# yenanjing/mmEgo

Measured on AMD Instinct MI355X. Metric: train frames/sec (Upper+Lower U+L step, B=64/GPU, T=8, 128 pts), higher is better.
Workload: dtype f32; 1 GPU; U+L step (Train_Upper + Train_Lower train_once bodies), B=64/GPU T=8 N=128, fp32, dropout live, two concurrent HIP-graph branches; global_batch=64, seq_len=8, points=128, parallelism=dp1

## Files before the change

mmego_amd/csrc/gemm.hip:

```cpp
#include <stdlib.h>

#include "common.h"

#include "gemm_tile.h"
#include "lstm_cell.h"
#include "tile_order.h"

struct GemmP {
  const float* A;
  const float* B;
  float* C;
  const float* bias;
  long sam, sak, sbk, sbn, scm, scn;
  long sAb, sBb, sCb, sCs, sBiasb;
  int M, N, K;
  int nsplit, kchunk;
  int relu, accumulate;
  int avec, bvec;
  const float* cmul;
  float* asum;
  const float* cb_dout[2]; long cb_dos;
  const float* cb_gst[2]; const float* cb_cst[2]; const float* cb_cprev[2];
  float* cb_dc[2]; float* cb_dg[2]; long cb_dgs;
};

#define LD64 68
constexpr long GEMM_TILE_MIN_OTHER = 256;
constexpr int GEMM_KQ_MAX = 512;

template <bool A_KC, bool B_KC, int BK>
__global__ __launch_bounds__(256) void gemm64_kernel(GemmP p) {
  constexpr int EL = BK / 4;
  __shared__ float As[BK][LD64];
  __shared__ float Bs[BK][LD64];
  const int tid = threadIdx.x, lane = tid & 63, wave = tid >> 6;
  const int wm = wave & 1, wn = wave >> 1;
  const int batch = blockIdx.z / p.nsplit, split = blockIdx.z % p.nsplit;
  const int m0 = blockIdx.x * 64, n0 = blockIdx.y * 64;
  const float* A = p.A + (long)batch * p.sAb;
  const float* B = p.B + (long)batch * p.sBb;
  const int kbeg = split * p.kchunk;
  const int kend = min(p.K, kbeg + p.kchunk);

  const int am = A_KC ? (tid >> 2) : (tid & 63), bn = B_KC ? (tid >> 2) : (tid & 63);
  const int akb = A_KC ? (tid & 3) * 4 : (tid >> 6), bkb = B_KC ? (tid & 3) * 4 : (tid >> 6);
  const float* Arow = A + (long)min(m0 + am, p.M - 1) * p.sam;
  const float* Bcol = B + (long)min(n0 + bn, p.N - 1) * p.sbn;
  const bool avec = A_KC && p.avec, bvec = B_KC && p.bvec;

  float ra[EL], rb[EL];
#define G64_PIN(v) asm volatile("" : "+v"(v))
#define G64_LOAD1(R, PTR, SK, KC, VEC, KB, k0)                                                                \
  do {                                                                                                        \
    const bool whole_ = (k0) + BK <= kend;                                                       \
    if (KC) {                                                                                                 \
      if ((VEC) && whole_) {                                                                                  \
        _Pragma("unroll") for (int g = 0; g < EL / 4; ++g) {                                                  \
          const f32x4 v = *reinterpret_cast<const f32x4*>((PTR) + (k0) + (KB) + 16 * g);                      \
          R[4 * g] = v.x; R[4 * g + 1] = v.y; R[4 * g + 2] = v.z; R[4 * g + 3] = v.w;                         \
        }                                                                                                     \
      } else {                                                                                                \
        _Pragma("unroll") for (int j = 0; j < EL; ++j)                                                        \
          R[j] = (PTR)[(long)min((k0) + (KB) + 16 * (j >> 2) + (j & 3), kend - 1) * (SK)];                    \
        if (!whole_) {                                                                                        \
          _Pragma("unroll") for (int j = 0; j < EL; ++j) {                                                    \
            G64_PIN(R[j]);                                                                                    \
            R[j] = ((k0) + (KB) + 16 * (j >> 2) + (j & 3) < kend) ? R[j] : 0.0f;                              \
          }                                                                                                   \
        }                                                                                                     \
      }                                                                                                       \
    } else {                                                                                                  \
      _Pragma("unroll") for (int j = 0; j < EL; ++j) R[j] = (PTR)[(long)min((k0) + (KB) + 4 * j, kend - 1) * (SK)]; \
      if (!whole_) {                                                                                          \
        _Pragma("unroll") for (int j = 0; j < EL; ++j) {                                                      \
          G64_PIN(R[j]);                                                                                      \
          R[j] = ((k0) + (KB) + 4 * j < kend) ? R[j] : 0.0f;                                                  \
        }                                                                                                     \
      }                                                                                                       \
    }                                                                                                         \
  } while (0)
#define G64_LOAD(k0)                                                                                          \
  do {                                                                                                        \
    G64_LOAD1(ra, Arow, p.sak, A_KC, avec, akb, k0);                                                          \
    G64_LOAD1(rb, Bcol, p.sbk, B_KC, bvec, bkb, k0);                                                          \
  } while (0)

  f32x16 acc = {0};
  if (kbeg < kend) G64_LOAD(kbeg);
  for (int k0 = kbeg; k0 < kend; k0 += BK) {
    __syncthreads();
#pragma unroll
    for (int j = 0; j < EL; ++j) {
      As[A_KC ? akb + 16 * (j >> 2) + (j & 3) : akb + 4 * j][am] = ra[j];
      Bs[B_KC ? bkb + 16 * (j >> 2) + (j & 3) : bkb + 4 * j][bn] = rb[j];
    }
    __syncthreads();
    if (k0 + BK < kend) G64_LOAD(k0 + BK);
    const int r = lane & 31, h = lane >> 5;
#pragma unroll
    for (int kk = 0; kk < BK; kk += 2) {
      float a = As[kk + h][wm * 32 + r];
      float b = Bs[kk + h][wn * 32 + r];
      acc = __builtin_amdgcn_mfma_f32_32x32x2f32(a, b, acc, 0, 0, 0);
    }
  }
#undef G64_LOAD
#undef G64_LOAD1
#undef G64_PIN

  const int col = n0 + wn * 32 + (lane & 31);
  if (col >= p.N) return;
  float* C = p.C + (long)batch * p.sCb + (long)split * p.sCs;
  const float bv = (p.bias && p.nsplit == 1) ? p.bias[(long)batch * p.sBiasb + col] : 0.0f;
  const int rbase = m0 + wm * 32 + 4 * (lane >> 5);
  const bool final_ = p.nsplit == 1;
  float old[16], cm[16];
  if (final_ && p.accumulate) {
#pragma unroll
    for (int reg = 0; reg < 16; ++reg) {
      const int row = rbase + (reg & 3) + 8 * (reg >> 2);
      old[reg] = C[(long)(row < p.M ? row : p.M - 1) * p.scm + (long)col * p.scn];
    }
  }
  if (final_ && p.cmul) {
    const float* cmp = p.cmul + (C - p.C);
#pragma unroll
    for (int reg = 0; reg < 16; ++reg) {
      const int row = rbase + (reg & 3) + 8 * (reg >> 2);
      cm[reg] = cmp[(long)(row < p.M ? row : p.M - 1) * p.scm + (long)col * p.scn];
    }
  }
#pragma unroll
  for (int reg = 0; reg < 16; ++reg) {
    float v = acc[reg] + bv;
    if (final_) {
      if (p.relu == 1) v = fmaxf(v, 0.0f);
      if (p.accumulate) { asm volatile("" : "+v"(old[reg])); v += old[reg]; }
      if (p.cmul) { asm volatile("" : "+v"(cm[reg])); v = p.relu == 2 ? (cm[reg] > 0.f ? v : 0.f) : v * cm[reg]; }
    }
    acc[reg] = v;
  }
  float* cp = C + (long)rbase * p.scm + (long)col * p.scn;
  if (m0 + wm * 32 + 32 <= p.M) {
#pragma unroll
    for (int reg = 0; reg < 16; ++reg) cp[(long)((reg & 3) + 8 * (reg >> 2)) * p.scm] = acc[reg];
  } else {
#pragma unroll
    for (int reg = 0; reg < 16; ++reg)
      if (rbase + (reg & 3) + 8 * (reg >> 2) < p.M) cp[(long)((reg & 3) + 8 * (reg >> 2)) * p.scm] = acc[reg];
  }
}

template <bool A_KC, bool B_KC>
__device__ __forceinline__ void gemm32kq_body(const GemmP& p, const int bx, const int by, const int bz) {
  __shared__ float red[4][32][33];
  const int tid = threadIdx.x, lane = tid & 63, wave = tid >> 6;
  const int r = lane & 31, h = lane >> 5;
  const int batch = bz / p.nsplit, split = bz % p.nsplit;
  const int m0 = bx * 32, n0 = by * 32;
  const float* A = p.A + (long)batch * p.sAb;
  const float* B = p.B + (long)batch * p.sBb;
  const int kbeg0 = split * p.kchunk;
  const int kend0 = min(p.K, kbeg0 + p.kchunk);
  const int kq = (((kend0 - kbeg0) + 3) / 4 + 31) / 32 * 32;
  const int kbeg = kbeg0 + wave * kq;
  const int kend = min(kend0, kbeg + kq);
  const float* Arow = A + (long)min(m0 + r, p.M - 1) * p.sam;
  const float* Bcol = B + (long)min(n0 + r, p.N - 1) * p.sbn;
  const bool avec = A_KC && p.avec, bvec = B_KC && p.bvec;

  float ra[16], rb[16], na[16], nb[16];
#define KQ_PIN(v) asm volatile("" : "+v"(v))
#define KQ_LOAD1(R, PTR, SK, VEC, k0)                                                                         \
  do {                                                                                                        \
    const int kl = (k0) + 16 * h;                                                                             \
    if ((VEC) && (k0) + 32 <= kend) {                                                                         \
      _Pragma("unroll") for (int g = 0; g < 4; ++g) {                                                         \
        const f32x4 v = *reinterpret_cast<const f32x4*>((PTR) + kl + 4 * g);                                  \
        R[4 * g] = v.x; R[4 * g + 1] = v.y; R[4 * g + 2] = v.z; R[4 * g + 3] = v.w;                           \
      }                                                                                                       \
    } else {                                                                                                  \
      _Pragma("unroll") for (int s_ = 0; s_ < 16; ++s_) R[s_] = (PTR)[(long)min(kl + s_, kend - 1) * (SK)];   \
      if ((k0) + 32 > kend) {                                                                                 \
        _Pragma("unroll") for (int s_ = 0; s_ < 16; ++s_) { KQ_PIN(R[s_]); R[s_] = (kl + s_ < kend) ? R[s_] : 0.0f; } \
      }                                                                                                       \
    }                                                                                                         \
  } while (0)
#define KQ_LOAD(RA, RB, k0)                                                                                   \
  do {                                                                                                        \
    KQ_LOAD1(RA, Arow, p.sak, avec, k0);                                                                      \
    KQ_LOAD1(RB, Bcol, p.sbk, bvec, k0);                                                                      \
  } while (0)

  f32x16 acc = {0};
  const bool want_asum = p.asum != nullptr && by == 0;
  float asum = 0.f;
  if (kbeg < kend) {
    KQ_LOAD(ra, rb, kbeg);
    for (int k0 = kbeg; k0 < kend; k0 += 32) {
      const bool more = k0 + 32 < kend;
      if (more) KQ_LOAD(na, nb, k0 + 32);
      if (want_asum) {
#pragma unroll
        for (int s_ = 0; s_ < 16; ++s_) asum += ra[s_];
      }
#pragma unroll
      for (int s_ = 0; s_ < 16; ++s_) acc = __builtin_amdgcn_mfma_f32_32x32x2f32(ra[s_], rb[s_], acc, 0, 0, 0);
      if (more) {
#pragma unroll
        for (int s_ = 0; s_ < 16; ++s_) { ra[s_] = na[s_]; rb[s_] = nb[s_]; }
      }
    }
  }
#undef KQ_LOAD
#undef KQ_LOAD1
#undef KQ_PIN
#pragma unroll
  for (int reg = 0; reg < 16; ++reg) red[wave][(reg & 3) + 8 * (reg >> 2) + 4 * h][r] = acc[reg];
  __shared__ float ared[4][2][32];
  if (want_asum) ared[wave][h][r] = asum;
  __syncthreads();
  if (want_asum && tid < 32 && m0 + tid < p.M) {
    float v = 0.f;
#pragma unroll
    for (int w = 0; w < 4; ++w) v += ared[w][0][tid] + ared[w][1][tid];
    if (p.nsplit == 1) {
      float* dst = p.asum + (long)batch * p.M + m0 + tid;
      *dst = p.accumulate ? *dst + v : v;
    } else {
      p.asum[((long)split * (gridDim.z / p.nsplit) + batch) * p.M + m0 + tid] = v;
    }
  }
  if (p.cb_dg[0]) {
    const int col = tid & 31, H = p.N, d = batch;
    float dh[4], gi[4], gf[4], gg[4], go[4], cc[4], cp[4], dcin[4];
#pragma unroll
    for (int e = 0; e < 4; ++e) {
      const int row = (tid >> 5) + 8 * e;
      const long r = m0 + row, j = n0 + col, i = r * H + j;
      const float rec = ((red[0][row][col] + red[1][row][col]) + red[2][row][col]) + red[3][row][col];
      const float* gs = p.cb_gst[d] + r * 4 * H + j;
      dh[e] = p.cb_dout[d][r * p.cb_dos + j] + rec;
      gi[e] = gs[0]; gf[e] = gs[H]; gg[e] = gs[2 * H]; go[e] = gs[3 * H];
      cc[e] = p.cb_cst[d][i];
      cp[e] = p.cb_cprev[d] ? p.cb_cprev[d][i] : 0.f;
      dcin[e] = p.cb_dc[d][i];
    }
    LstmCellGrad o[4];
#pragma unroll
    for (int e = 0; e < 4; ++e) {
      asm volatile("" : "+v"(gi[e]), "+v"(gf[e]), "+v"(gg[e]), "+v"(go[e]), "+v"(cc[e]), "+v"(cp[e]), "+v"(dcin[e]), "+v"(dh[e]));
      o[e] = lstm_cell_bwd(gi[e], gf[e], gg[e], go[e], tanhf(cc[e]), cp[e], dcin[e], dh[e]);
    }
#pragma unroll
    for (int e = 0; e < 4; ++e) {
      const int row = (tid >> 5) + 8 * e;
      const long r = m0 + row, j = n0 + col;
      float* dg = p.cb_dg[d] + r * p.cb_dgs + j;
      dg[0] = o[e].di; dg[H] = o[e].df; dg[2 * H] = o[e].dg; dg[3 * H] = o[e].dout;
      p.cb_dc[d][r * H + j] = o[e].dcprev;
    }
    return;
  }
  float* C = p.C + (long)batch * p.sCb + (long)split * p.sCs;
  const bool final_ = p.nsplit == 1;
  const int col = tid & 31, colc = n0 + col < p.N ? n0 + col : p.N - 1;
  long off[4];
  float v[4], old[4], cm[4], bv = 0.f;
#pragma unroll
  for (int e = 0; e < 4; ++e) {
    const int row = (tid >> 5) + 8 * e;
    v[e] = ((red[0][row][col] + red[1][row][col]) + red[2][row][col]) + red[3][row][col];
    off[e] = (long)(m0 + row < p.M ? m0 + row : p.M - 1) * p.scm + (long)colc * p.scn;
  }
  if (final_ && p.bias) bv = p.bias[(long)batch * p.sBiasb + colc];
  if (final_ && p.accumulate) {
#pragma unroll
    for (int e = 0; e < 4; ++e) old[e] = C[off[e]];
  }
  if (final_ && p.cmul) {
    const float* cmp = p.cmul + (C - p.C);
#pragma unroll
    for (int e = 0; e < 4; ++e) cm[e] = cmp[off[e]];
  }
  if (final_) {
#pragma unroll
    for (int e = 0; e < 4; ++e) {
      float x = v[e] + bv;
      if (p.relu == 1) x = fmaxf(x, 0.0f);
      if (p.accumulate) { asm volatile("" : "+v"(old[e])); x += old[e]; }
      if (p.cmul) { asm volatile("" : "+v"(cm[e])); x = p.relu == 2 ? (cm[e] > 0.f ? x : 0.f) : x * cm[e]; }
      v[e] = x;
    }
  }
  if (m0 + 32 <= p.M && n0 + 32 <= p.N) {
#pragma unroll
    for (int e = 0; e < 4; ++e) C[off[e]] = v[e];
  } else {
#pragma unroll
    for (int e = 0; e < 4; ++e)
      if (m0 + (tid >> 5) + 8 * e < p.M && n0 + col < p.N) C[off[e]] = v[e];
  }
}

template <bool A_KC, bool B_KC>
__global__ __launch_bounds__(256) void gemm32kq_kernel(GemmP p) {
  gemm32kq_body<A_KC, B_KC>(p, blockIdx.x, blockIdx.y, blockIdx.z);
}

#define GEMM_GROUP_MAX 10
struct GemmGroup { GemmP p[GEMM_GROUP_MAX]; int zend[GEMM_GROUP_MAX]; int n; };
template <bool A_KC, bool B_KC>
__global__ __launch_bounds__(256) void gemm32kq_group_kernel(GemmGroup g) {
  int i = 0;
  const int z = blockIdx.z;
  while (i + 1 < g.n && z >= g.zend[i]) ++i;
  const int z0 = i ? g.zend[i - 1] : 0;
  const GemmP& p = g.p[i];
  if ((int)blockIdx.x * 32 >= p.M || (int)blockIdx.y * 32 >= p.N) return;
  gemm32kq_body<A_KC, B_KC>(p, blockIdx.x, blockIdx.y, z - z0);
}

#define SKR_OUT 16
#define SKR_LANES 16
__global__ __launch_bounds__(256) void splitk_reduce_kernel(const float* __restrict__ ws, float* C, const float* bias, int nsplit,
                                                            int nbatch, int M, int N, long scm, long scn, long sCb,
                                                            int relu, int accumulate, const float* __restrict__ asum_ws,
                                                            float* asum_out) {
  __shared__ float sh[SKR_LANES][SKR_OUT + 1];
  long total = (long)nbatch * M * N;
  const int o = threadIdx.x & (SKR_OUT - 1), kg = threadIdx.x / SKR_OUT;
  long i = (long)blockIdx.x * SKR_OUT + o;
  const long cblocks = (total + SKR_OUT - 1) / SKR_OUT;
  const bool is_asum = (long)blockIdx.x >= cblocks;
  if (is_asum) {
    i = ((long)blockIdx.x - cblocks) * SKR_OUT + o;
    total = (long)nbatch * M;
    ws = asum_ws;
  }
  float s = 0.0f;
  if (i < total) {
    const float* src = ws + i;
    int k = kg;
#pragma unroll 1
    for (; k + 7 * SKR_LANES < nsplit; k += 8 * SKR_LANES) {
      float v[8];
#pragma unroll
      for (int u = 0; u < 8; ++u) v[u] = src[(long)(k + u * SKR_LANES) * total];
#pragma unroll
      for (int u = 0; u < 8; ++u) s += v[u];
    }
    for (; k < nsplit; k += SKR_LANES) s += src[(long)k * total];
  }
  sh[kg][o] = s;
  __syncthreads();
  if (kg == 0 && i < total) {
    s = sh[0][o];
#pragma unroll
    for (int g = 1; g < SKR_LANES; ++g) s += sh[g][o];
    if (is_asum) {
      asum_out[i] = accumulate ? asum_out[i] + s : s;
      return;
    }
    int n = (int)(i % N);
    long r = i / N;
    int m = (int)(r % M);
    int b = (int)(r / M);
    if (bias) s += bias[n];
    if (relu) s = fmaxf(s, 0.0f);
    float* dst = C + (long)b * sCb + (long)m * scm + (long)n * scn;
    if (accumulate) s += *dst;
    *dst = s;
  }
}

#define LD128 132

__global__ __launch_bounds__(256) void gemm128_nt_kernel(const float* __restrict__ A, const float* __restrict__ W,
                                                         float* __restrict__ C, const float* __restrict__ bias,
                                                         int M, int N, int K, long lda, long ldw, long ldc, int relu) {
  __shared__ float As[2][16][LD128];
  __shared__ float Bs[2][16][LD128];
  const int tid = threadIdx.x, lane = tid & 63, wave = tid >> 6;
  const int wm = wave & 1, wn = wave >> 1;
  const int ntn = N / 128, ntm = M / 128;
  const int id = xcd_order(blockIdx.x, ntn * ntm);
  const int m0 = (id / ntn) * 128, n0 = (id % ntn) * 128;

  const int lr = tid >> 2, lk = (tid & 3) * 4;
  const float* Ap = A + (long)(m0 + lr) * lda + lk;
  const float* Wp = W + (long)(n0 + lr) * ldw + lk;
  float4 ra[2], rb[2];
  auto gload = [&](int k0) {
    ra[0] = *reinterpret_cast<const float4*>(Ap + k0);
    ra[1] = *reinterpret_cast<const float4*>(Ap + 64 * lda + k0);
    rb[0] = *reinterpret_cast<const float4*>(Wp + k0);
    rb[1] = *reinterpret_cast<const float4*>(Wp + 64 * ldw + k0);
  };
  auto sstore = [&](int buf) {
#pragma unroll
    for (int h = 0; h < 2; ++h) {
      As[buf][lk + 0][lr + 64 * h] = ra[h].x; As[buf][lk + 1][lr + 64 * h] = ra[h].y;
      As[buf][lk + 2][lr + 64 * h] = ra[h].z; As[buf][lk + 3][lr + 64 * h] = ra[h].w;
      Bs[buf][lk + 0][lr + 64 * h] = rb[h].x; Bs[buf][lk + 1][lr + 64 * h] = rb[h].y;
      Bs[buf][lk + 2][lr + 64 * h] = rb[h].z; Bs[buf][lk + 3][lr + 64 * h] = rb[h].w;
    }
  };

  f32x16 acc[2][2];
#pragma unroll
  for (int i = 0; i < 2; ++i)
#pragma unroll
    for (int j = 0; j < 2; ++j) acc[i][j] = (f32x16){0};

  const int nk = K / 16;
  gload(0);
  sstore(0);
  __syncthreads();
  const int r = lane & 31, h = lane >> 5;
  for (int kt = 0; kt < nk; ++kt) {
    const int buf = kt & 1;
    if (kt + 1 < nk) gload((kt + 1) * 16);
#pragma unroll
    for (int kk = 0; kk < 16; kk += 2) {
      float a0 = As[buf][kk + h][wm * 64 + r], a1 = As[buf][kk + h][wm * 64 + 32 + r];
      float b0 = Bs[buf][kk + h][wn * 64 + r], b1 = Bs[buf][kk + h][wn * 64 + 32 + r];
      acc[0][0] = __builtin_amdgcn_mfma_f32_32x32x2f32(a0, b0, acc[0][0], 0, 0, 0);
      acc[0][1] = __builtin_amdgcn_mfma_f32_32x32x2f32(a0, b1, acc[0][1], 0, 0, 0);
      acc[1][0] = __builtin_amdgcn_mfma_f32_32x32x2f32(a1, b0, acc[1][0], 0, 0, 0);
      acc[1][1] = __builtin_amdgcn_mfma_f32_32x32x2f32(a1, b1, acc[1][1], 0, 0, 0);
    }
    if (kt + 1 < nk) sstore(buf ^ 1);
    __syncthreads();
  }

#pragma unroll
  for (int j = 0; j < 2; ++j) {
    const int col = n0 + wn * 64 + j * 32 + (lane & 31);
    const float bv = bias ? bias[col] : 0.0f;
#pragma unroll
    for (int i = 0; i < 2; ++i) {
#pragma unroll
      for (int reg = 0; reg < 16; ++reg) {
        int row = m0 + wm * 64 + i * 32 + (reg & 3) + 8 * (reg >> 2) + 4 * (lane >> 5);
        float v = acc[i][j][reg] + bv;
        if (relu) v = fmaxf(v, 0.0f);
        C[(long)row * ldc + col] = v;
      }
    }
  }
}

extern "C" int mmego_gemm(void* stream, const float* A, long sam, long sak, const float* B, long sbk, long sbn,
                          float* C, long scm, long scn, const float* bias, int M, int N, int K, int nbatch, long sAb,
                          long sBb, long sCb, int relu, int accumulate, float* splitk_ws, int nsplit, long sBiasb,
                          const float* cmul, float* asum) {
  MMEGO_REQUIRE(A && B && C && M > 0 && N > 0 && K > 0 && nbatch > 0 && nsplit >= 1);
  const bool defer = accumulate == 2;
  MMEGO_REQUIRE(!defer || (nsplit > 1 && nbatch == 1 && !bias && !relu));
  MMEGO_REQUIRE(!cmul || nsplit == 1);
  MMEGO_REQUIRE(relu == 0 || relu == 1 || (relu == 2 && cmul));
  MMEGO_REQUIRE(sBiasb == 0 || nsplit == 1);
  hipStream_t st = (hipStream_t)stream;
  {
    const bool a_kc = sak == 1, a_mc = sam == 1 && !a_kc;
    const bool b_kc = sbk == 1, b_mc = sbn == 1 && !b_kc;
    const long lda = a_kc ? sam : sak, ldw = b_kc ? sbn : sbk;
    const int kchunk_t = nsplit > 1 ? cdiv(cdiv(K, nsplit), 64) * 64 : K;
    constexpr long tile_min_other = GEMM_TILE_MIN_OTHER;
    const long tile_min_units = (a_kc && b_kc && nsplit == 1) ? (K <= 1024 ? 1 : 200) : tile_min_other;
    const long units64 = (long)(M / 64) * (N / 64) * nsplit * nbatch;
    const bool ok = !cmul && !asum && scn == 1 && (nbatch == 1 || ((sAb % 4) == 0 && (sBb % 4) == 0)) && (a_kc || a_mc) && (b_kc || b_mc) && (lda % 4) == 0 && (ldw % 4) == 0 &&
                    (((uintptr_t)A | (uintptr_t)B) & 15) == 0 && (M % 64) == 0 && (N % 64) == 0 &&
                    (K % 64) == 0 && units64 >= tile_min_units && (nsplit == 1 || (long)(nsplit - 1) * kchunk_t < K);
    if (ok) {
      TileP tp;
      tp.A = A; tp.W = B; tp.C = C; tp.bias = bias;
      tp.M = M; tp.N = N; tp.K = K;
      tp.lda = lda; tp.ldw = ldw; tp.ldc = scm;
      tp.relu = relu; tp.accumulate = accumulate;
      tp.nsplit = nsplit; tp.kchunk = kchunk_t; tp.ws = splitk_ws;
      tp.nbatch = nbatch; tp.sAb = sAb; tp.sWb = sBb; tp.sCb = sCb; tp.sBiasb = sBiasb;
      int rc = mmego_detail::gemm_tile_launch(st, tp, a_kc, b_kc);
      if (rc == 0 && nsplit > 1 && !defer) {
        long total = (long)nbatch * M * N;
        int blocks = (int)((total + SKR_OUT - 1) / SKR_OUT);
        hipLaunchKernelGGL(splitk_reduce_kernel, dim3(blocks), dim3(256), 0, st, splitk_ws, C, bias, nsplit, nbatch, M, N, scm, scn,
                           sCb, relu, accumulate, (const float*)nullptr, (float*)nullptr);
        MMEGO_LAUNCH_CHECK();
      }
      if (rc != -2) return rc;
    }
  }
  const bool fast = !cmul && !asum && nbatch == 1 && nsplit == 1 && !accumulate && sak == 1 && sbk == 1 && scn == 1 && (M % 128) == 0 &&
                    (N % 128) == 0 && (K % 16) == 0 && (sam % 4) == 0 && (sbn % 4) == 0 &&
                    (((uintptr_t)A | (uintptr_t)B) & 15) == 0;
  if (fast) {
    dim3 grid((M / 128) * (N / 128));
    hipLaunchKernelGGL(gemm128_nt_kernel, grid, dim3(256), 0, st, A, B, C, bias, M, N, K, sam, sbn, scm, relu);
    MMEGO_LAUNCH_CHECK();
    return MMEGO_OK;
  }
  GemmP p;
  p.A = A; p.B = B; p.bias = bias;
  p.sam = sam; p.sak = sak; p.sbk = sbk; p.sbn = sbn;
  p.sAb = sAb; p.sBb = sBb; p.sBiasb = sBiasb;
  p.M = M; p.N = N; p.K = K;
  p.nsplit = nsplit;
  p.relu = relu; p.accumulate = accumulate;
  p.cmul = cmul;
  p.asum = asum;
  p.cb_dg[0] = p.cb_dg[1] = nullptr;
  if (nsplit > 1) {
    MMEGO_REQUIRE(splitk_ws != nullptr);
    int kc = cdiv(K, nsplit);
    p.kchunk = cdiv(kc, 16) * 16;
    p.C = splitk_ws; p.scm = N; p.scn = 1; p.sCb = (long)M * N; p.sCs = (long)nbatch * M * N;
    if (asum) p.asum = splitk_ws + (long)nsplit * nbatch * M * N;
  } else {
    p.kchunk = cdiv(K, 16) * 16;
    p.C = C; p.scm = scm; p.scn = scn; p.sCb = sCb; p.sCs = 0;
  }
  MMEGO_REQUIRE(cdiv(N, 32) <= 65535 && (long)nbatch * nsplit <= 65535);
  const long wgs64 = (long)cdiv(M, 64) * cdiv(N, 64) * nbatch * nsplit;
  constexpr int kq_max = GEMM_KQ_MAX;
  const bool kq = wgs64 <= kq_max && p.kchunk >= 64;
  MMEGO_REQUIRE(!asum || kq);
  dim3 grid(cdiv(M, kq ? 32 : 64), cdiv(N, kq ? 32 : 64), nbatch * nsplit);
  const bool akc = (sak == 1), bkc = (sbk == 1);
  p.avec = akc && (sam % 4) == 0 && (sAb % 4) == 0 && ((uintptr_t)A & 15) == 0;
  p.bvec = bkc && (sbn % 4) == 0 && (sBb % 4) == 0 && ((uintptr_t)B & 15) == 0;
  const bool deep = p.kchunk >= 64;
#define G64_LAUNCH(AK, BKC)                                                                        \
  do {                                                                                             \
    if (kq) hipLaunchKernelGGL((gemm32kq_kernel<AK, BKC>), grid, dim3(256), 0, st, p);             \
    else if (deep) hipLaunchKernelGGL((gemm64_kernel<AK, BKC, 64>), grid, dim3(256), 0, st, p);    \
    else hipLaunchKernelGGL((gemm64_kernel<AK, BKC, 16>), grid, dim3(256), 0, st, p);              \
  } while (0)
  if (akc && bkc) G64_LAUNCH(true, true);
  else if (akc) G64_LAUNCH(true, false);
  else if (bkc) G64_LAUNCH(false, true);
  else G64_LAUNCH(false, false);
#undef G64_LAUNCH
  MMEGO_LAUNCH_CHECK();
  if (nsplit > 1 && !defer) {
    long total = (long)nbatch * M * N;
    int blocks = (int)((total + SKR_OUT - 1) / SKR_OUT);
    if (asum) blocks += (int)(((long)nbatch * M + SKR_OUT - 1) / SKR_OUT);
    hipLaunchKernelGGL(splitk_reduce_kernel, dim3(blocks), dim3(256), 0, st, splitk_ws, C, bias, nsplit, nbatch, M, N,
                       scm, scn, sCb, relu, accumulate, (const float*)p.asum, asum);
    MMEGO_LAUNCH_CHECK();
  }
  return MMEGO_OK;
}

int lstm_bwd_step_dma_try(void* stream, int Bn, int H, const float* dg0, const float* dg1, long dgs, const float* wT0,
                                           const float* wT1, const float* dout0, const float* dout1, long dos, const float* gst0,
                                           const float* gst1, const float* cst0, const float* cst1, const float* cprev0,
                                           const float* cprev1, float* dc0, float* dc1, float* dgo0, float* dgo1);

extern "C" int mmego_lstm_bwd_step(void* stream, int Bn, int H, const float* dg0, const float* dg1, long dgs, const float* wT0,
                                   const float* wT1, const float* dout0, const float* dout1, long dos, const float* gst0,
                                   const float* gst1, const float* cst0, const float* cst1, const float* cprev0,
                                   const float* cprev1, float* dc0, float* dc1, float* dgo0, float* dgo1) {
  MMEGO_REQUIRE(Bn > 0 && H > 0 && (Bn % 32) == 0 && (H % 32) == 0 && dg0 && dg1 && wT0 && wT1 && dout0 && dout1 && gst0 && gst1 &&
                cst0 && cst1 && dc0 && dc1 && dgo0 && dgo1 && (cprev0 == nullptr) == (cprev1 == nullptr));
  MMEGO_REQUIRE((dgs % 4) == 0 && ((((uintptr_t)dg0) | ((uintptr_t)dg1) | ((uintptr_t)wT0) | ((uintptr_t)wT1)) & 15) == 0);
  {
    const int rc = lstm_bwd_step_dma_try(stream, Bn, H, dg0, dg1, dgs, wT0, wT1, dout0, dout1, dos, gst0, gst1, cst0, cst1,
                                               cprev0, cprev1, dc0, dc1, dgo0, dgo1);
    if (rc != -1) return rc;
  }
  GemmP p;
  p.A = dg0; p.B = wT0; p.C = nullptr; p.bias = nullptr;
  p.sam = dgs; p.sak = 1; p.sbk = 1; p.sbn = 4L * H;
  p.sAb = dg1 - dg0; p.sBb = wT1 - wT0; p.sBiasb = 0;
  p.scm = H; p.scn = 1; p.sCb = 0; p.sCs = 0;
  p.M = Bn; p.N = H; p.K = 4 * H;
  p.nsplit = 1; p.kchunk = cdiv(p.K, 16) * 16;
  p.relu = 0; p.accumulate = 0;
  p.cmul = nullptr; p.asum = nullptr;
  p.avec = (p.sAb % 4) == 0; p.bvec = (p.sBb % 4) == 0;
  p.cb_dout[0] = dout0; p.cb_dout[1] = dout1; p.cb_dos = dos;
  p.cb_gst[0] = gst0; p.cb_gst[1] = gst1; p.cb_cst[0] = cst0; p.cb_cst[1] = cst1;
  p.cb_cprev[0] = cprev0; p.cb_cprev[1] = cprev1;
  p.cb_dc[0] = dc0; p.cb_dc[1] = dc1; p.cb_dg[0] = dgo0; p.cb_dg[1] = dgo1; p.cb_dgs = dgs;
  dim3 grid(Bn / 32, H / 32, 2);
  hipLaunchKernelGGL((gemm32kq_kernel<true, true>), grid, dim3(256), 0, (hipStream_t)stream, p);
  MMEGO_LAUNCH_CHECK();
  return MMEGO_OK;
}

extern "C" int mmego_gemm_group(void* stream, int n, const MmegoGemmDesc* d) {
  MMEGO_REQUIRE(n >= 1 && d);
  constexpr long tile_min_other = GEMM_TILE_MIN_OTHER;
  constexpr int kq_max = GEMM_KQ_MAX;
  bool ok = n >= 2 && n <= GEMM_GROUP_MAX;
  const bool akc = d[0].sak == 1, bkc = d[0].sbk == 1;
  GemmGroup g;
  unsigned gx = 0, gy = 0;
  int z = 0;
  for (int i = 0; ok && i < n; ++i) {
    const MmegoGemmDesc& a = d[i];
    if (!(a.A && a.B && a.C && a.M > 0 && a.N > 0 && a.K > 0 && a.nbatch > 0)) return MMEGO_EBADARG;
    const long units64 = (long)(a.M / 64) * (a.N / 64) * a.nbatch;
    const long wgs64 = (long)cdiv(a.M, 64) * cdiv(a.N, 64) * a.nbatch;
    ok = a.nsplit == 1 && (a.sak == 1) == akc && (a.sbk == 1) == bkc && !(akc && bkc) && units64 < tile_min_other &&
         wgs64 <= kq_max && a.K >= 64 && a.relu != 2 && cdiv(a.N, 32) <= 65535;
    if (!ok) break;
    GemmP& p = g.p[i];
    p.A = a.A; p.B = a.B; p.bias = a.bias;
    p.sam = a.sam; p.sak = a.sak; p.sbk = a.sbk; p.sbn = a.sbn;
    p.sAb = a.sAb; p.sBb = a.sBb; p.sBiasb = a.sBiasb;
    p.M = a.M; p.N = a.N; p.K = a.K;
    p.nsplit = 1; p.kchunk = cdiv(a.K, 16) * 16;
    p.relu = a.relu; p.accumulate = a.accumulate;
    p.cmul = a.cmul; p.asum = a.asum;
    p.cb_dg[0] = p.cb_dg[1] = nullptr;
    p.C = a.C; p.scm = a.scm; p.scn = a.scn; p.sCb = a.sCb; p.sCs = 0;
    p.avec = akc && (a.sam % 4) == 0 && (a.sAb % 4) == 0 && ((uintptr_t)a.A & 15) == 0;
    p.bvec = bkc && (a.sbn % 4) == 0 && (a.sBb % 4) == 0 && ((uintptr_t)a.B & 15) == 0;
    const unsigned tx = (unsigned)cdiv(a.M, 32), ty = (unsigned)cdiv(a.N, 32);
    gx = tx > gx ? tx : gx; gy = ty > gy ? ty : gy;
    z += a.nbatch;
    g.zend[i] = z;
  }
  if (!ok || z > 65535) {
    for (int i = 0; i < n; ++i) {
      const MmegoGemmDesc& a = d[i];
      int rc = mmego_gemm(stream, a.A, a.sam, a.sak, a.B, a.sbk, a.sbn, a.C, a.scm, a.scn, a.bias, a.M, a.N, a.K, a.nbatch, a.sAb, a.sBb,
                          a.sCb, a.relu, a.accumulate, a.splitk_ws, a.nsplit, a.sBiasb, a.cmul, a.asum);
      if (rc != MMEGO_OK) return rc;
    }
    return MMEGO_OK;
  }
  g.n = n;
  for (int i = n; i < GEMM_GROUP_MAX; ++i) g.zend[i] = z;
  dim3 grid(gx, gy, (unsigned)z);
  hipStream_t st = (hipStream_t)stream;
  if (akc) hipLaunchKernelGGL((gemm32kq_group_kernel<true, false>), grid, dim3(256), 0, st, g);
  else if (bkc) hipLaunchKernelGGL((gemm32kq_group_kernel<false, true>), grid, dim3(256), 0, st, g);
  else hipLaunchKernelGGL((gemm32kq_group_kernel<false, false>), grid, dim3(256), 0, st, g);
  MMEGO_LAUNCH_CHECK();
  return MMEGO_OK;
}
```

mmego_amd/csrc/gemm_tile.hip:

```cpp
#include <stdlib.h>

#include "common.h"
#include "gemm_tile.h"
#include "lds_dma.h"
#include "tile_order.h"

#define TLD_MAX 68

template <int BM, int BN, int WAVES_M, int WAVES_N, bool A_KC, bool B_KC, int KCH>
__device__ __forceinline__ void gemm_tile_body(const TileP& p, int m0, int n0, int sb, float* smem, int sid) {
  const int split = sb % p.nsplit, batch = sb / p.nsplit;
  static_assert(WAVES_M * WAVES_N == 4, "4 waves");
  static_assert(KCH == 64 || KCH == 32, "k per staged chunk");
  constexpr int TLD = KCH + 4;
  constexpr int WM = BM / WAVES_M, WN = BN / WAVES_N;
  constexpr int TM = WM / 32, TN = WN / 32;
  constexpr int AV = BM * KCH / 1024, BV = BN * KCH / 1024;
  constexpr int LPR = KCH / 4, RPP = 256 / LPR;
  constexpr int ALD = BM + 4, BLD = BN + 4;
  constexpr int ARP = 1024 / BM, BRP = 1024 / BN;
  float* As = smem;
  float* Bs = smem + BM * TLD;
  const int tid = threadIdx.x, lane = tid & 63, wave = tid >> 6;
  const int wm = wave % WAVES_M, wn = wave / WAVES_M;
  const int kbeg = split * p.kchunk, kend = min(p.K, kbeg + p.kchunk);
  const int nk = (kend - kbeg) / KCH;

  const int lk = (tid % LPR) * 4, lr = tid / LPR;
  const int amk = tid / (BM / 4), am4 = (tid % (BM / 4)) * 4;
  const int bnk = tid / (BN / 4), bn4 = (tid % (BN / 4)) * 4;
  const float* Ab = p.A + (long)batch * p.sAb;
  const float* Wb = p.W + (long)batch * p.sWb;
  const float* Ap = A_KC ? Ab + (long)(m0 + lr) * p.lda + kbeg + lk : Ab + (long)(kbeg + amk) * p.lda + m0 + am4;
  const float* Wp = B_KC ? Wb + (long)(n0 + lr) * p.ldw + kbeg + lk : Wb + (long)(kbeg + bnk) * p.ldw + n0 + bn4;
  const long astep = A_KC ? RPP * p.lda : (long)ARP * p.lda, akstep = A_KC ? KCH : KCH * p.lda;
  const long bstep = B_KC ? RPP * p.ldw : (long)BRP * p.ldw, bkstep = B_KC ? KCH : KCH * p.ldw;
  f32x4 ra[AV], rb[BV];
  f32x16 acc[TM][TN];
#pragma unroll
  for (int i = 0; i < TM; ++i)
#pragma unroll
    for (int j = 0; j < TN; ++j) acc[i][j] = (f32x16){0};

  MMEGO_STAMP_AT(sid, 0, tid == 0);
  if (nk > 0) {
#pragma unroll
    for (int i = 0; i < AV; ++i) ra[i] = *reinterpret_cast<const f32x4*>(Ap + i * astep);
#pragma unroll
    for (int i = 0; i < BV; ++i) rb[i] = *reinterpret_cast<const f32x4*>(Wp + i * bstep);
  }
  const int r = lane & 31, h = lane >> 5;
  MMEGO_STAMP_AT(sid, 1, tid == 0);
  for (int kt = 0; kt < nk; ++kt) {
    __syncthreads();
#pragma unroll
    for (int i = 0; i < AV; ++i) {
      if (A_KC) *reinterpret_cast<f32x4*>(&As[(lr + RPP * i) * TLD + lk]) = ra[i];
      else *reinterpret_cast<f32x4*>(&As[(amk + ARP * i) * ALD + am4]) = ra[i];
    }
#pragma unroll
    for (int i = 0; i < BV; ++i) {
      if (B_KC) *reinterpret_cast<f32x4*>(&Bs[(lr + RPP * i) * TLD + lk]) = rb[i];
      else *reinterpret_cast<f32x4*>(&Bs[(bnk + BRP * i) * BLD + bn4]) = rb[i];
    }
    __syncthreads();
    if (kt + 1 < nk) {
      const float* An = Ap + (kt + 1) * akstep;
      const float* Wn = Wp + (kt + 1) * bkstep;
#pragma unroll
      for (int i = 0; i < AV; ++i) ra[i] = *reinterpret_cast<const f32x4*>(An + i * astep);
#pragma unroll
      for (int i = 0; i < BV; ++i) rb[i] = *reinterpret_cast<const f32x4*>(Wn + i * bstep);
    }
#pragma unroll
    for (int kb = 0; kb < KCH / 8; ++kb) {
      f32x4 a[TM], b[TN];
#pragma unroll
      for (int i = 0; i < TM; ++i) {
        if (A_KC) {
          a[i] = *reinterpret_cast<const f32x4*>(&As[(wm * WM + i * 32 + r) * TLD + kb * 8 + 4 * h]);
        } else {
          const float* q = &As[(kb * 8 + 4 * h) * ALD + wm * WM + i * 32 + r];
          a[i] = (f32x4){q[0], q[ALD], q[2 * ALD], q[3 * ALD]};
        }
      }
#pragma unroll
      for (int j = 0; j < TN; ++j) {
        if (B_KC) {
          b[j] = *reinterpret_cast<const f32x4*>(&Bs[(wn * WN + j * 32 + r) * TLD + kb * 8 + 4 * h]);
        } else {
          const float* q = &Bs[(kb * 8 + 4 * h) * BLD + wn * WN + j * 32 + r];
          b[j] = (f32x4){q[0], q[BLD], q[2 * BLD], q[3 * BLD]};
        }
      }
#pragma unroll
      for (int i = 0; i < TM; ++i)
#pragma unroll
        for (int j = 0; j < TN; ++j) acc[i][j] = __builtin_amdgcn_mfma_f32_32x32x2f32(a[i].x, b[j].x, acc[i][j], 0, 0, 0);
#pragma unroll
      for (int i = 0; i < TM; ++i)
#pragma unroll
        for (int j = 0; j < TN; ++j) acc[i][j] = __builtin_amdgcn_mfma_f32_32x32x2f32(a[i].y, b[j].y, acc[i][j], 0, 0, 0);
#pragma unroll
      for (int i = 0; i < TM; ++i)
#pragma unroll
        for (int j = 0; j < TN; ++j) acc[i][j] = __builtin_amdgcn_mfma_f32_32x32x2f32(a[i].z, b[j].z, acc[i][j], 0, 0, 0);
#pragma unroll
      for (int i = 0; i < TM; ++i)
#pragma unroll
        for (int j = 0; j < TN; ++j) acc[i][j] = __builtin_amdgcn_mfma_f32_32x32x2f32(a[i].w, b[j].w, acc[i][j], 0, 0, 0);
    }
  }
  MMEGO_STAMP_AT(sid, 2, tid == 0);

  const bool slab = p.nsplit > 1;
  float* C = slab ? p.ws + ((long)split * p.nbatch + batch) * p.M * p.N : p.C + (long)batch * p.sCb;
  const long ldc = slab ? (long)p.N : p.ldc;
  const bool relu = !slab && p.relu, accumulate = !slab && p.accumulate;
#pragma unroll
  for (int j = 0; j < TN; ++j) {
    const int col = n0 + wn * WN + j * 32 + (lane & 31);
    const float bv = (!slab && p.bias) ? p.bias[(long)batch * p.sBiasb + col] : 0.0f;
#pragma unroll
    for (int i = 0; i < TM; ++i) {
      float* cp = C + (long)(m0 + wm * WM + i * 32 + 4 * (lane >> 5)) * ldc + col;
      float old[16];
      if (accumulate) {
#pragma unroll
        for (int reg = 0; reg < 16; ++reg) old[reg] = cp[(long)((reg & 3) + 8 * (reg >> 2)) * ldc];
#pragma unroll
        for (int reg = 0; reg < 16; ++reg) asm volatile("" : "+v"(old[reg]));
      }
#pragma unroll
      for (int reg = 0; reg < 16; ++reg) {
        float v = acc[i][j][reg] + bv;
        if (relu) v = fmaxf(v, 0.0f);
        if (accumulate) v += old[reg];
        cp[(long)((reg & 3) + 8 * (reg >> 2)) * ldc] = v;
      }
    }
  }
  MMEGO_STAMP_AT(sid, 3, tid == 0);
}

template <int BM, int BN, int WAVES_M, int WAVES_N, bool A_KC, bool B_KC, int KCH>
__global__ __launch_bounds__(256) void gemm_tile_kernel(TileP p) {
  extern __shared__ __attribute__((aligned(16))) float smem[];
  const int ntn = p.N / BN, tiles = ntn * (p.M / BM);
  const int u = xcd_order(blockIdx.x, (int)gridDim.x);
  const int split = u / tiles, id = u % tiles;
  gemm_tile_body<BM, BN, WAVES_M, WAVES_N, A_KC, B_KC, KCH>(p, (id / ntn) * BM, (id % ntn) * BN, split, smem, u);
}

template <bool A_KC, bool B_KC, int KCH>
__global__ __launch_bounds__(256) void gemm_tile_persistent_kernel(TileP p, int nfull, int nhalf, int stagger) {
  extern __shared__ __attribute__((aligned(16))) float smem[];
  const int ntn = p.N / 128, tiles = ntn * (p.M / 128), G = (int)gridDim.x;
  const int w = xcd_order(blockIdx.x, G);
  const bool halves_first = (int)blockIdx.x >= G / 2 && stagger;
  if (halves_first)
    for (int q = w; q < nhalf; q += G) {
      const int u = nfull + (q >> 1), id = u % tiles;
      gemm_tile_body<128, 64, 2, 2, A_KC, B_KC, KCH>(p, (id / ntn) * 128, (id % ntn) * 128 + (q & 1) * 64, u / tiles, smem, nfull + q);
    }
  for (int u = w; u < nfull; u += G) {
    const int id = u % tiles;
    gemm_tile_body<128, 128, 2, 2, A_KC, B_KC, KCH>(p, (id / ntn) * 128, (id % ntn) * 128, u / tiles, smem, u);
  }
  if (!halves_first)
    for (int q = w; q < nhalf; q += G) {
      const int u = nfull + (q >> 1), id = u % tiles;
      gemm_tile_body<128, 64, 2, 2, A_KC, B_KC, KCH>(p, (id / ntn) * 128, (id % ntn) * 128 + (q & 1) * 64, u / tiles, smem, nfull + q);
    }
}

struct TileBigArgs {
  int tiles_m, tiles_n;
};

template <int DUMMY>
__global__ __launch_bounds__(512, 1) void gemm_tile_big_kernel(TileP p, TileBigArgs g) {
  constexpr int BM = 320, BN = 256, KCH = 32, ROWS = BM + BN, STAGE = ROWS * KCH;
  extern __shared__ __attribute__((aligned(16))) float smem[];
  const int tid = threadIdx.x, lane = tid & 63;
  const int w = __builtin_amdgcn_readfirstlane(tid >> 6);
  const int wm = w >> 2, wn = w & 3;
  const TileMN t = panel_walk_or_row_major(blockIdx.x, gridDim.x, g.tiles_m, g.tiles_n);
  const int batch = t.m / g.tiles_m;
  const int m0 = (t.m - batch * g.tiles_m) * BM, n0 = t.n * BN;
  const int kbeg = p.nsplit > 1 ? (int)blockIdx.y * p.kchunk : 0;
  const int kend = p.nsplit > 1 ? min(p.K, kbeg + p.kchunk) : p.K;
  const float* Ab = p.A + (long)batch * p.sAb + (long)m0 * p.lda + kbeg;
  const float* Wb = p.W + (long)batch * p.sWb + (long)n0 * p.ldw + kbeg;
  const float* gp[9];
#pragma unroll
  for (int j = 0; j < 9; ++j) {
    const int i = w + 8 * j;
    const bool isw = i >= BM / 8;
    const int row = (isw ? i - BM / 8 : i) * 8 + (lane >> 3);
    const int piece = (lane & 7) ^ ((row >> 1) & 7);
    gp[j] = (isw ? Wb + (long)row * p.ldw : Ab + (long)row * p.lda) + 4 * piece;
  }
#ifndef GTB_EXP
#define GTB_EXP 0
#endif
#define GTB_DMA(kt, stage)                                                                                                  \
  if (!((GTB_EXP & 1) && (kt) > 1)) {                                                                                       \
    _Pragma("unroll") for (int j = 0; j < 9; ++j)                                                                           \
      GLDS16(gp[j] + (long)(kt) * KCH, smem + (stage) * STAGE + (w + 8 * j) * 8 * KCH);                                     \
  }
  const int nk = (kend - kbeg) / KCH;
  const int r = lane & 31, h = lane >> 5, key = (r >> 1) & 7;
  int off[4];
#pragma unroll
  for (int kb = 0; kb < 4; ++kb) off[kb] = r * KCH + 4 * ((2 * kb + h) ^ key);
  f32x16 acc[5][2];
#pragma unroll
  for (int i = 0; i < 5; ++i)
#pragma unroll
    for (int j = 0; j < 2; ++j) acc[i][j] = (f32x16){0};
  GTB_DMA(0, 0)
  if (nk > 1) GTB_DMA(1, 1)
  asm volatile("s_waitcnt vmcnt(0)" ::: "memory");
  __builtin_amdgcn_s_barrier();
#ifndef GTB_SCHED
#define GTB_SCHED 1
#endif
#if GTB_SCHED == 1
#define GTB_USE(x) asm volatile("" ::"v"(x))
#define GTB_SB() __builtin_amdgcn_sched_barrier(0)
  f32x4 a[5], b[2][2];
  {
    const float* As = smem + wm * 160 * KCH;
    const float* Bs = smem + (BM + wn * 64) * KCH;
#pragma unroll
    for (int i = 0; i < 3; ++i) a[i] = *reinterpret_cast<const f32x4*>(As + i * 32 * KCH + off[0]);
#pragma unroll
    for (int j = 0; j < 2; ++j) b[0][j] = *reinterpret_cast<const f32x4*>(Bs + j * 32 * KCH + off[0]);
  }
  for (int kt = 0; kt < nk; ++kt) {
#pragma unroll
    for (int kb = 0; kb < 4; ++kb) {
      const float* Ac = smem + (kt & 1) * STAGE + wm * 160 * KCH + off[kb];
      const int nst = kb < 3 ? (kt & 1) : ((kt + 1) & 1);
      const float* An = smem + nst * STAGE + wm * 160 * KCH + off[(kb + 1) & 3];
      const float* Bn = smem + nst * STAGE + (BM + wn * 64) * KCH + off[(kb + 1) & 3];
      const bool more = kb < 3 || kt + 1 < nk;
#pragma unroll
      for (int i = 0; i < 5; ++i) {
        GTB_USE(a[i]);
        if (i == 0) { GTB_USE(b[kb & 1][0]); GTB_USE(b[kb & 1][1]); }
        GTB_SB();
        if (i == 2 && kb == 3) {
          asm volatile("s_waitcnt vmcnt(0) lgkmcnt(0)" ::: "memory");
          __builtin_amdgcn_s_barrier();
          if (kt + 2 < nk) GTB_DMA(kt + 2, kt & 1)
        }
        if (i < 2) a[i + 3] = *reinterpret_cast<const f32x4*>(Ac + (i + 3) * 32 * KCH);
        else if (more) a[i - 2] = *reinterpret_cast<const f32x4*>(An + (i - 2) * 32 * KCH);
        if (i == 2 && more) {
#pragma unroll
          for (int j = 0; j < 2; ++j) b[(kb + 1) & 1][j] = *reinterpret_cast<const f32x4*>(Bn + j * 32 * KCH);
        }
        GTB_SB();
#pragma unroll
        for (int c = 0; c < 4; ++c)
#pragma unroll
          for (int j = 0; j < 2; ++j) acc[i][j] = __builtin_amdgcn_mfma_f32_32x32x2f32(a[i][c], b[kb & 1][j][c], acc[i][j], 0, 0, 0);
        GTB_SB();
      }
    }
  }
#undef GTB_USE
#undef GTB_SB
#else
  f32x4 a[5], b[2];
  for (int kt = 0; kt < nk; ++kt) {
    const float* As = smem + (kt & 1) * STAGE + wm * 160 * KCH;
    const float* Bs = smem + (kt & 1) * STAGE + (BM + wn * 64) * KCH;
#pragma unroll
    for (int kb = 0; kb < 4; ++kb) {
      if (!(GTB_EXP & 2) || (kt == 0 && kb == 0)) {
#pragma unroll
        for (int i = 0; i < 5; ++i) a[i] = *reinterpret_cast<const f32x4*>(As + i * 32 * KCH + off[kb]);
#pragma unroll
        for (int j = 0; j < 2; ++j) b[j] = *reinterpret_cast<const f32x4*>(Bs + j * 32 * KCH + off[kb]);
      }
      if (kb == 3) {
        asm volatile("s_waitcnt vmcnt(0) lgkmcnt(0)" ::: "memory");
        __builtin_amdgcn_s_barrier();
        if (kt + 2 < nk) GTB_DMA(kt + 2, kt & 1)
      }
#pragma unroll
      for (int c = 0; c < 4; ++c)
#pragma unroll
        for (int i = 0; i < 5; ++i)
#pragma unroll
          for (int j = 0; j < 2; ++j) acc[i][j] = __builtin_amdgcn_mfma_f32_32x32x2f32(a[i][c], b[j][c], acc[i][j], 0, 0, 0);
    }
  }
#endif
#undef GTB_DMA
  const bool slabs = p.nsplit > 1;
  float* C = slabs ? p.ws + (long)blockIdx.y * p.M * p.N : p.C + (long)batch * p.sCb;
  const long ldc = slabs ? (long)p.N : p.ldc;
#pragma unroll
  for (int j = 0; j < 2; ++j) {
    const int col = n0 + wn * 64 + j * 32 + r;
    const float bv = (p.bias && !slabs) ? p.bias[(long)batch * p.sBiasb + col] : 0.0f;
#pragma unroll
    for (int i = 0; i < 5; ++i) {
      float* cp = C + (long)(m0 + wm * 160 + i * 32 + 4 * h) * ldc + col;
#pragma unroll
      for (int reg = 0; reg < 16; ++reg)
        if (!(GTB_EXP & 4) || acc[i][j][reg] == 12345.f) cp[(long)((reg & 3) + 8 * (reg >> 2)) * ldc] = acc[i][j][reg] + bv;
    }
  }
}

namespace mmego_detail {

constexpr int GT_KCH = 32;

template <int BM, int BN, bool A_KC, bool B_KC, int KCH>
static int launch_plain_k(hipStream_t st, const TileP& p) {
  const size_t lds = (size_t)((BM + BN) * (KCH + 4)) * sizeof(float);
  if (int e = mmego_allow_lds<gemm_tile_kernel<BM, BN, 2, 2, A_KC, B_KC, KCH>>(lds)) return e;
  const unsigned units = (unsigned)((p.M / BM) * (p.N / BN) * p.nsplit * p.nbatch);
  hipLaunchKernelGGL((gemm_tile_kernel<BM, BN, 2, 2, A_KC, B_KC, KCH>), dim3(units), dim3(256), lds, st, p);
  hipError_t e = hipGetLastError();
  return e == hipSuccess ? 0 : (int)e;
}

template <int BM, int BN, bool A_KC, bool B_KC>
static int launch_plain(hipStream_t st, const TileP& p) { return launch_plain_k<BM, BN, A_KC, B_KC, GT_KCH>(st, p); }

template <bool A_KC, bool B_KC>
static int launch_layout(hipStream_t st, const TileP& p) {
  if (A_KC && B_KC) {
    static const bool big = !(getenv("MMEGO_GEMM_BIG") && atoi(getenv("MMEGO_GEMM_BIG")) == 0);
    const long tiles = (long)(p.M / 320) * (p.N / 256) * p.nbatch;
    const bool slab_ok = p.nsplit == 1 ? !p.accumulate
                                       : (p.accumulate == 2 && p.nbatch == 1 && p.ws && !p.bias && (p.kchunk % 32) == 0 && p.kchunk >= 64 &&
                                          (long)(p.nsplit - 1) * p.kchunk < p.K && (p.K - (long)(p.nsplit - 1) * p.kchunk) >= 64);
    const long units = tiles * p.nsplit;
    if (big && (p.M % 320) == 0 && (p.N % 256) == 0 && (p.K % 32) == 0 && p.K >= 64 && slab_ok && !p.relu &&
        units >= 256 && (units % 256) == 0 && tiles < (1L << 30) && (p.lda % 4) == 0 && (p.ldw % 4) == 0 && (p.sAb % 4) == 0 && (p.sWb % 4) == 0 &&
        ((((uintptr_t)p.A) | ((uintptr_t)p.W)) & 15) == 0) {
      constexpr int lds = 2 * (320 + 256) * 32 * (int)sizeof(float);
      if (int e = mmego_allow_lds<gemm_tile_big_kernel<0>>(lds)) return e;
      TileBigArgs g = {p.M / 320, p.N / 256};
      hipLaunchKernelGGL((gemm_tile_big_kernel<0>), dim3((unsigned)tiles, (unsigned)p.nsplit), dim3(512), lds, st, p, g);
      hipError_t e = hipGetLastError();
      return e == hipSuccess ? 0 : (int)e;
    }
  }
  const long units128 = (long)(p.M / 128) * (p.N / 128) * p.nsplit * p.nbatch;
  const bool big_ok = (p.M % 128) == 0 && (p.N % 128) == 0 && units128 >= 192;
  if (big_ok) {
    static const int slots = getenv("MMEGO_GEMM_SLOTS") ? atoi(getenv("MMEGO_GEMM_SLOTS")) : 512;
    const int units = (int)units128;
    if (units > slots && p.K > 128) {
      const int rest = units % slots;
      const bool halves = rest > 0 && rest <= slots / 2;
      const int nfull = halves ? units - rest : units, nhalf = halves ? 2 * rest : 0;
      const size_t lds = slots <= 256 ? 84 * 1024 : (size_t)(256 * (GT_KCH + 4)) * sizeof(float);
      if (int e = mmego_allow_lds<gemm_tile_persistent_kernel<A_KC, B_KC, GT_KCH>>(lds)) return e;
      hipLaunchKernelGGL((gemm_tile_persistent_kernel<A_KC, B_KC, GT_KCH>), dim3(slots), dim3(256), lds, st, p, nfull, nhalf, 1);
      hipError_t e = hipGetLastError();
      return e == hipSuccess ? 0 : (int)e;
    }
    return launch_plain<128, 128, A_KC, B_KC>(st, p);
  }
  return launch_plain<64, 64, A_KC, B_KC>(st, p);
}

int gemm_tile_launch(hipStream_t st, const TileP& p, bool a_kc, bool b_kc) {
  if ((p.K % 64) != 0 || (p.M % 64) != 0 || (p.N % 64) != 0 || p.nsplit < 1 || p.nbatch < 1) return -2;
  if (p.nsplit > 1 && ((p.kchunk % 64) != 0 || p.ws == nullptr)) return -2;
  if (a_kc && b_kc) return launch_layout<true, true>(st, p);
  if (a_kc) return launch_layout<true, false>(st, p);
  if (b_kc) return launch_layout<false, true>(st, p);
  return launch_layout<false, false>(st, p);
}

}
```

Before: 104,900 frames/s.

## Add 64x128 LDS-DMA GEMM tile kernel for mid-size K-contiguous GEMMs

Adds a new 64x128 tile GEMM kernel that stages A and W chunks into LDS via direct global-to-LDS loads with a multi-stage counted-wait pipeline and swizzled LDS layout, using fp32 MFMA. It is selected for K-contiguous, non-split GEMMs that are too small for the 128x128 paths but still fill the CUs, replacing the plain 64x64 kernel there. The tile path is also opened to K divisible by 32 (not just 64), routing such shapes away from the fallback GEMM. Risks include more register/LDS pressure and correctness of the wait counts for odd chunk counts.

```diff
diff --git a/mmego_amd/csrc/gemm.hip b/mmego_amd/csrc/gemm.hip
--- a/mmego_amd/csrc/gemm.hip
+++ b/mmego_amd/csrc/gemm.hip
@@ -472,7 +472,7 @@
     const long units64 = (long)(M / 64) * (N / 64) * nsplit * nbatch;
     const bool ok = !cmul && !asum && scn == 1 && (nbatch == 1 || ((sAb % 4) == 0 && (sBb % 4) == 0)) && (a_kc || a_mc) && (b_kc || b_mc) && (lda % 4) == 0 && (ldw % 4) == 0 &&
                     (((uintptr_t)A | (uintptr_t)B) & 15) == 0 && (M % 64) == 0 && (N % 64) == 0 &&
-                    (K % 64) == 0 && units64 >= tile_min_units && (nsplit == 1 || (long)(nsplit - 1) * kchunk_t < K);
+                    ((K % 64) == 0 || (a_kc && b_kc && nsplit == 1 && (K % 32) == 0)) && units64 >= tile_min_units && (nsplit == 1 || (long)(nsplit - 1) * kchunk_t < K);
     if (ok) {
       TileP tp;
       tp.A = A; tp.W = B; tp.C = C; tp.bias = bias;
diff --git a/mmego_amd/csrc/gemm_tile.hip b/mmego_amd/csrc/gemm_tile.hip
--- a/mmego_amd/csrc/gemm_tile.hip
+++ b/mmego_amd/csrc/gemm_tile.hip
@@ -318,6 +318,143 @@
   }
 }
 
+template <int NST>
+__global__ __launch_bounds__(256) void gemm_tile_dma64_kernel(TileP p) {
+  constexpr int BM = 64, BN = 128, KCH = 32, TN = BN / 64, ROWS = BM + BN, STAGE = ROWS * KCH;
+  constexpr int PW = ROWS / 8 / 4;
+  static_assert(NST >= 2 && NST <= 4, "the counted waits below cover up to 3 chunks in flight behind the one waited for");
+  extern __shared__ __attribute__((aligned(16))) float smem[];
+  const int tid = threadIdx.x, lane = tid & 63;
+  const int w = __builtin_amdgcn_readfirstlane(tid >> 6);
+  const int wm = w >> 1, wn = w & 1;
+  const int tiles_m = p.M / BM, tiles = tiles_m * (p.N / BN);
+  const int u = xcd_order(blockIdx.x, (int)gridDim.x);
+  const int batch = u / tiles, id = u - batch * tiles;
+  const int m0 = (id % tiles_m) * BM, n0 = (id / tiles_m) * BN;
+  const float* Ab = p.A + (long)batch * p.sAb + (long)m0 * p.lda;
+  const float* Wb = p.W + (long)batch * p.sWb + (long)n0 * p.ldw;
+  const float* gp[PW];
+#pragma unroll
+  for (int j = 0; j < PW; ++j) {
+    const bool isw = j >= BM / 32;
+    const int row = (w + 4 * j - (isw ? BM / 8 : 0)) * 8 + (lane >> 3);
+    const int piece = (lane & 7) ^ ((row >> 1) & 7);
+    gp[j] = (isw ? Wb + (long)row * p.ldw : Ab + (long)row * p.lda) + 4 * piece;
+  }
+#ifndef GTD_EXP
+#define GTD_EXP 0
+#endif
+#define GTD_DMA(kt, stage)                                                                                                  \
+  {                                                                                                                         \
+    _Pragma("unroll") for (int j = 0; j < PW; ++j)                                                                          \
+      GLDS16(gp[j] + (long)(kt) * KCH, smem + (stage) * STAGE + (w + 4 * j) * 8 * KCH);                                     \
+  }
+#define GTD_WAIT(ahead)                                                                                                     \
+  {                                                                                                                         \
+    if ((ahead) >= 3) wait_vmcnt<3 * PW>();                                                                                 \
+    else if ((ahead) == 2) wait_vmcnt<2 * PW>();                                                                            \
+    else if ((ahead) == 1) wait_vmcnt<PW>();                                                                                \
+    else wait_vmcnt<0>();                                                                                                   \
+  }
+#define GTD_BARRIER()                                                                                                       \
+  {                                                                                                                         \
+    asm volatile("" ::: "memory");                                                                                          \
+    __builtin_amdgcn_s_barrier();                                                                                           \
+    asm volatile("" ::: "memory");                                                                                          \
+  }
+#define GTD_USE(x) asm volatile("" ::"v"(x))
+#define GTD_SB() __builtin_amdgcn_sched_barrier(0)
+  const int nk = p.K / KCH;
+  const int r = lane & 31, h = lane >> 5, key = (r >> 1) & 7;
+  int off[4];
+#pragma unroll
+  for (int kb = 0; kb < 4; ++kb) off[kb] = r * KCH + 4 * ((2 * kb + h) ^ key);
+  const int aoff = wm * 32 * KCH, boff = (BM + wn * (BN / 2)) * KCH;
+  f32x16 acc[TN];
+#pragma unroll
+  for (int j = 0; j < TN; ++j) acc[j] = (f32x16){0};
+  MMEGO_STAMP_AT(u, 0, tid == 0);
+#pragma unroll
+  for (int c = 0; c < NST; ++c)
+    if (c < nk) GTD_DMA(c, c)
+  GTD_WAIT(min(nk, NST) - 1)
+  GTD_BARRIER()
+  f32x4 a[2], b[2][TN];
+  a[0] = *reinterpret_cast<const f32x4*>(smem + aoff + off[0]);
+#pragma unroll
+  for (int j = 0; j < TN; ++j) b[0][j] = *reinterpret_cast<const f32x4*>(smem + boff + j * 32 * KCH + off[0]);
+  MMEGO_STAMP_AT(u, 1, tid == 0);
+  int cur = 0;
+  for (int kt = 0; kt < nk; ++kt) {
+    const int nxt = cur + 1 == NST ? 0 : cur + 1;
+    const float* Sc = smem + cur * STAGE;
+    const float* Sn = smem + nxt * STAGE;
+#pragma unroll
+    for (int kb = 0; kb < 4; ++kb) {
+      const int q = kb & 1;
+      GTD_USE(a[q]);
+#pragma unroll
+      for (int j = 0; j < TN; ++j) GTD_USE(b[q][j]);
+      GTD_SB();
+      if (kb < 3) {
+        if (!(GTD_EXP & 2)) {
+          a[q ^ 1] = *reinterpret_cast<const f32x4*>(Sc + aoff + off[(kb + 1) & 3]);
+#pragma unroll
+          for (int j = 0; j < TN; ++j) b[q ^ 1][j] = *reinterpret_cast<const f32x4*>(Sc + boff + j * 32 * KCH + off[(kb + 1) & 3]);
+        }
+        GTD_SB();
+#pragma unroll
+        for (int c = 0; c < 4; ++c)
+#pragma unroll
+          for (int j = 0; j < TN; ++j) acc[j] = __builtin_amdgcn_mfma_f32_32x32x2f32(a[q][c], b[q][j][c], acc[j], 0, 0, 0);
+      } else {
+#pragma unroll
+        for (int c = 0; c < 2; ++c)
+#pragma unroll
+          for (int j = 0; j < TN; ++j) acc[j] = __builtin_amdgcn_mfma_f32_32x32x2f32(a[q][c], b[q][j][c], acc[j], 0, 0, 0);
+        GTD_SB();
+        if (kt + 1 < nk) {
+          GTD_WAIT(min(kt + NST, nk) - kt - 2)
+          GTD_BARRIER()
+          if (!(GTD_EXP & 1) && kt + NST < nk) GTD_DMA(kt + NST, cur)
+          if (!(GTD_EXP & 2)) {
+            a[q ^ 1] = *reinterpret_cast<const f32x4*>(Sn + aoff + off[0]);
+#pragma unroll
+            for (int j = 0; j < TN; ++j) b[q ^ 1][j] = *reinterpret_cast<const f32x4*>(Sn + boff + j * 32 * KCH + off[0]);
+          }
+        }
+        GTD_SB();
+#pragma unroll
+        for (int c = 2; c < 4; ++c)
+#pragma unroll
+          for (int j = 0; j < TN; ++j) acc[j] = __builtin_amdgcn_mfma_f32_32x32x2f32(a[q][c], b[q][j][c], acc[j], 0, 0, 0);
+      }
+      GTD_SB();
+    }
+    cur = nxt;
+  }
+  MMEGO_STAMP_AT(u, 2, tid == 0);
+#undef GTD_DMA
+#undef GTD_WAIT
+#undef GTD_BARRIER
+#undef GTD_USE
+#undef GTD_SB
+  float* C = p.C + (long)batch * p.sCb;
+#pragma unroll
+  for (int j = 0; j < TN; ++j) {
+    const int col = n0 + wn * (BN / 2) + j * 32 + r;
+    const float bv = p.bias ? p.bias[(long)batch * p.sBiasb + col] : 0.0f;
+    float* cp = C + (long)(m0 + wm * 32 + 4 * h) * p.ldc + col;
+#pragma unroll
+    for (int reg = 0; reg < 16; ++reg) {
+      float v = acc[j][reg] + bv;
+      if (p.relu) v = fmaxf(v, 0.0f);
+      cp[(long)((reg & 3) + 8 * (reg >> 2)) * p.ldc] = v;
+    }
+  }
+  MMEGO_STAMP_AT(u, 3, tid == 0);
+}
+
 namespace mmego_detail {
 
 constexpr int GT_KCH = 32;
@@ -335,9 +472,26 @@
 template <int BM, int BN, bool A_KC, bool B_KC>
 static int launch_plain(hipStream_t st, const TileP& p) { return launch_plain_k<BM, BN, A_KC, B_KC, GT_KCH>(st, p); }
 
+static bool dma64_fits(const TileP& p) {
+  return (p.M % 64) == 0 && (p.N % 128) == 0 && (p.K % 32) == 0 && p.nsplit == 1 && !p.accumulate && (p.relu == 0 || p.relu == 1) &&
+         (long)(p.M / 64) * (p.N / 128) * p.nbatch < (1L << 30) && (p.lda % 4) == 0 && (p.ldw % 4) == 0 && (p.sAb % 4) == 0 && (p.sWb % 4) == 0 &&
+         ((((uintptr_t)p.A) | ((uintptr_t)p.W)) & 15) == 0;
+}
+
+template <int NST>
+static int launch_dma64(hipStream_t st, const TileP& p) {
+  constexpr int lds = NST * (64 + 128) * 32 * (int)sizeof(float);
+  if (int e = mmego_allow_lds<gemm_tile_dma64_kernel<NST>>(lds)) return e;
+  const unsigned tiles = (unsigned)((p.M / 64) * (p.N / 128) * p.nbatch);
+  hipLaunchKernelGGL((gemm_tile_dma64_kernel<NST>), dim3(tiles), dim3(256), lds, st, p);
+  hipError_t e = hipGetLastError();
+  return e == hipSuccess ? 0 : (int)e;
+}
+
 template <bool A_KC, bool B_KC>
 static int launch_layout(hipStream_t st, const TileP& p) {
-  if (A_KC && B_KC) {
+  const bool k64 = (p.K % 64) == 0;
+  if (A_KC && B_KC && k64) {
     static const bool big = !(getenv("MMEGO_GEMM_BIG") && atoi(getenv("MMEGO_GEMM_BIG")) == 0);
     const long tiles = (long)(p.M / 320) * (p.N / 256) * p.nbatch;
     const bool slab_ok = p.nsplit == 1 ? !p.accumulate
@@ -356,7 +510,7 @@
     }
   }
   const long units128 = (long)(p.M / 128) * (p.N / 128) * p.nsplit * p.nbatch;
-  const bool big_ok = (p.M % 128) == 0 && (p.N % 128) == 0 && units128 >= 192;
+  const bool big_ok = k64 && (p.M % 128) == 0 && (p.N % 128) == 0 && units128 >= 192;
   if (big_ok) {
     static const int slots = getenv("MMEGO_GEMM_SLOTS") ? atoi(getenv("MMEGO_GEMM_SLOTS")) : 512;
     const int units = (int)units128;
@@ -372,11 +526,26 @@
     }
     return launch_plain<128, 128, A_KC, B_KC>(st, p);
   }
+  if (A_KC && B_KC && dma64_fits(p)) {
+    const char* env = getenv("MMEGO_GEMM_DMA64");
+    const int mode = env ? atoi(env) : 1;
+    if ((mode & 2) || (long)(p.M / 64) * (p.N / 128) * p.nbatch >= mmego_cu_count()) {
+      if (!(mode & 1)) return launch_plain<64, 64, A_KC, B_KC>(st, p);
+#ifdef GTD_PROBE
+      const int var = getenv("MMEGO_GEMM_DMA64_VAR") ? atoi(getenv("MMEGO_GEMM_DMA64_VAR")) : 0;
+      if (var == 1) return launch_dma64<3>(st, p);
+      if (var == 2) return launch_dma64<4>(st, p);
+#endif
+      return launch_dma64<2>(st, p);
+    }
+  }
+  if ((p.K % 64) != 0) return -2;
   return launch_plain<64, 64, A_KC, B_KC>(st, p);
 }
 
 int gemm_tile_launch(hipStream_t st, const TileP& p, bool a_kc, bool b_kc) {
-  if ((p.K % 64) != 0 || (p.M % 64) != 0 || (p.N % 64) != 0 || p.nsplit < 1 || p.nbatch < 1) return -2;
+  const bool k_ok = (p.K % 64) == 0 || (a_kc && b_kc && p.nsplit == 1 && (p.K % 32) == 0);
+  if (!k_ok || (p.M % 64) != 0 || (p.N % 64) != 0 || p.nsplit < 1 || p.nbatch < 1) return -2;
   if (p.nsplit > 1 && ((p.kchunk % 64) != 0 || p.ws == nullptr)) return -2;
   if (a_kc && b_kc) return launch_layout<true, true>(st, p);
   if (a_kc) return launch_layout<true, false>(st, p);
```

Result: no change. 105,400 frames/s, median of 6 (+0.5%).
